# luuvish/arrow-h264

Measured on AMD Instinct MI355X. Metric: macroblocks/s (decode reconstruct, post-entropy) 1080p P-frame; % HBM roofline, higher is better.
Workload: dtype u8

## Files before the change

### arrow-h264_amd/csrc/k_deblock2.hip

```cpp
#include "kernels.h"
#include "mb_deblock.h"
#include "mb_deblock2.h"

using namespace h264r;

namespace {

constexpr int LPU = H264R_DB2_LPU;
static_assert(LPU == 4 || LPU == 8, "H264R_DB2_LPU");
constexpr int UNITS = DEBLOCK2_UNITS;
constexpr int NH = LPU / 4;
constexpr int BAND = H264R_DB2_BAND;
#ifndef H264R_DB2_PL
#define H264R_DB2_PL 2
#endif
constexpr int PL = H264R_DB2_PL;
constexpr bool DOY = PL != 1, DOC = PL != 0;
static_assert(PL == 2 || LPU == 8, "the split walk is built at 8 lanes per unit");
constexpr int PICS = UNITS / BAND;
#ifndef H264R_DB2_SG
#define H264R_DB2_SG 4
#endif
constexpr int SG = H264R_DB2_SG;
static_assert(SG == 4 || SG == 2, "H264R_DB2_SG");
static_assert(UNITS % BAND == 0, "a band divides the wave's units");
constexpr int RECG = 24;
static_assert(HANDOFF2_BYTES == 2 * RECG * sizeof(uint64_t), "the host sizes hb by HANDOFF2_BYTES per MB column");
constexpr int AUX_SC1 = 16;
constexpr int RSRC_W3 = 0x00020000;
constexpr uint32_t OOB = 0x80000000u;

constexpr int YR = DOY ? 16 : 0, CR = DOC ? 8 : 0;
struct alignas(16) UnitLds {
    uint32_t y[YR][8];
    uint32_t c[2][CR][4];
    uint32_t info[20];
};
static_assert(sizeof(UnitLds) == (PL == 2 ? 848 : PL == 0 ? 592 : 336), "UnitLds layout");

struct alignas(16) StageLds {
    uint32_t y[YR][SG][4];
    uint32_t c[2][CR][SG][2];
    uint32_t pad[SG == 4 ? 20 : 4];
};
static_assert(SG != 4 || sizeof(StageLds) == (PL == 2 ? 1616 : PL == 0 ? 1104 : 592), "StageLds layout");
struct alignas(16) UpLds {
    uint32_t yu[DOY ? 3 : 0][SG][4];
    uint32_t cu[2][DOC ? SG : 0][2];
};

typedef uint32_t v4u __attribute__((ext_vector_type(4)));
typedef uint32_t v2u __attribute__((ext_vector_type(2)));

DEV s2 unpack_cols(uint32_t w, int j) { return as_s2(__builtin_amdgcn_perm(w, w, 0x0C000C00u | ((uint32_t)(j + 2) << 16) | (uint32_t)j)); }
DEV uint32_t pack_cols(s2 c0, s2 c1) { return __builtin_amdgcn_perm(as_w(c1), as_w(c0), 0x06020400u); }
DEV s2 bs_pair(uint32_t w, int slo, int shi) { return (s2){(short)((w >> (8 * slo)) & 255), (short)((w >> (8 * shi)) & 255)}; }

template <int AUX = 0>
DEV void st16(__amdgpu_buffer_rsrc_t r, uint32_t off, v4u v)
{
    __builtin_amdgcn_raw_buffer_store_b128(__builtin_bit_cast(__attribute__((ext_vector_type(4))) unsigned int, v), r, off, 0, AUX);
}
template <int AUX = 0>
DEV void st8(__amdgpu_buffer_rsrc_t r, uint32_t off, v2u v)
{
    __builtin_amdgcn_raw_buffer_store_b64(__builtin_bit_cast(__attribute__((ext_vector_type(2))) unsigned int, v), r, off, 0, AUX);
}
template <int AUX = 0>
DEV void st4(__amdgpu_buffer_rsrc_t r, uint32_t off, uint32_t v) { __builtin_amdgcn_raw_buffer_store_b32(v, r, off, 0, AUX); }
#ifndef H264R_DB2_OUT_AUX
#define H264R_DB2_OUT_AUX 0
#endif
constexpr int OUT_AUX = H264R_DB2_OUT_AUX;

}

#ifndef H264R_DB2_KERNEL
#define H264R_DB2_KERNEL k_deblock2
#endif
#ifdef H264R_TRACE
#if H264R_DB2_PL == 0
#define h264r_db2_trace h264r_db2y_trace
#define h264r_db2_trace_copy h264r_db2y_trace_copy
#elif H264R_DB2_PL == 1
#define h264r_db2_trace h264r_db2c_trace
#define h264r_db2_trace_copy h264r_db2c_trace_copy
#endif
__device__ unsigned long long h264r_db2_trace[1 << 16][8];
#define TRACE(...) __VA_ARGS__
extern "C" void h264r_db2_trace_copy(void* dst) { (void)hipMemcpyFromSymbol(dst, HIP_SYMBOL(h264r_db2_trace), sizeof(h264r_db2_trace)); }
#else
#define TRACE(...)
#endif

#ifndef H264R_DB2_XCD
#define H264R_DB2_XCD 1
#endif
#ifndef H264R_DB2_DIAG
#define H264R_DB2_DIAG 0
#endif
#define H264R_DB2_WAVES_PER_EU (H264R_DB2_PL == 1 ? 4 : H264R_DB2_PL == 0 ? 3 : H264R_DB2_LPU == 8 ? (H264R_DB2_SG == 2 ? 3 : 2) : 1)
extern "C" __global__ __launch_bounds__(64) __attribute__((amdgpu_waves_per_eu(H264R_DB2_WAVES_PER_EU, H264R_DB2_WAVES_PER_EU))) void H264R_DB2_KERNEL(
    h264r_batch b, const DbInfo* __restrict__ dbinfo, uint64_t* hb, int* sync, int* err, uint32_t epoch, int2 rows, int nx,
    const uint8_t* __restrict__ recon)
{
    __shared__ UnitLds S[UNITS];
    __shared__ StageLds G[UNITS];
    __shared__ UpLds UP[PICS];
#ifdef H264R_DB2_LDS_PAD
    __shared__ uint32_t lds_pad[H264R_DB2_LDS_PAD / 4];
    if (threadIdx.x == 0 && epoch == 0xFFFFFFFFu) { lds_pad[0] = 1; __syncthreads(); err[0] = lds_pad[0]; }
#endif
    const Geom g = make_geom(b.width_mbs, b.height_mbs);
    const int W = g.wmb, R0 = rows.x, R1 = rows.y;
    const int ngroups = (b.num_pics + PICS - 1) / PICS;
    const int nbands = (R1 - R0 + BAND - 1) / BAND;
#if !H264R_DB2_XCD
    nx = 1;
#endif
    unsigned xcc_reg = 0;
    if (nx > 1) asm volatile("s_getreg_b32 %0, hwreg(HW_REG_XCC_ID)" : "=s"(xcc_reg));
    const int xcc = (int)(xcc_reg & 15u) % nx;
    const int ngx = (ngroups - xcc + nx - 1) / nx;
    int* counter = &sync[xcc];
    const bool local = nx > 1;
    const int items = ngx * nbands;
    for (;;) {
    __syncthreads();
    int tk = 0;
    if (threadIdx.x == 0) tk = atomicAdd(counter, 1);
    const int ticket = __builtin_amdgcn_readfirstlane(tk);
    if (ticket >= items) {
        xcd_drain_check(sync, sync + TICKET_DRAIN, nx, [&](int k) { return (ngroups - k + nx - 1) / nx * nbands; }, err);
        return;
    }
    const int band = ticket / ngx, grp = (ticket - band * ngx) * nx + xcc;
    int lane = threadIdx.x;
    asm volatile("" : "+v"(lane));
    const int u = lane / LPU, q8 = lane % LPU, q = q8 / NH, h = q8 % NH;
    const int rb = u / PICS, pu = u - rb * PICS;
    const int y = R0 + band * BAND + rb;
    const int pic0 = grp * PICS, npg = min(PICS, b.num_pics - pic0);
    const bool active = pu < npg && y < R1;
    const int pic = pic0 + min(pu, npg - 1), yc = min(y, R1 - 1);
    const bool above = y > R0, last_row = y == R1 - 1;
    const uint32_t tag32 = (epoch << 12) | ((uint32_t)band & 0xFFFu);
    const uint64_t tag_in = (uint64_t)((epoch << 12) | ((uint32_t)(band - 1) & 0xFFFu)) << 32;
    const bool polls = active && rb == 0 && above;
    const bool publishes = active && rb == BAND - 1 && !last_row;

    UnitLds& U = S[u];
    const UnitLds& A = S[rb ? u - PICS : u];
    StageLds& T = G[u];
    StageLds& TA = G[rb ? u - PICS : u];
    UpLds& TU = UP[pu];
    const uint32_t Wl = (uint32_t)g.W, Wc = (uint32_t)g.Wc;
    const uint32_t ysz = (uint32_t)g.ysz, csz = (uint32_t)g.csz;
    const __amdgpu_buffer_rsrc_t rY = __builtin_amdgcn_make_buffer_rsrc(b.out_y + (size_t)pic0 * g.ysz, 0, (int)(npg * ysz), RSRC_W3);
    const __amdgpu_buffer_rsrc_t rU = __builtin_amdgcn_make_buffer_rsrc(b.out_u + (size_t)pic0 * g.csz, 0, (int)(npg * csz), RSRC_W3);
    const __amdgpu_buffer_rsrc_t rV = __builtin_amdgcn_make_buffer_rsrc(b.out_v + (size_t)pic0 * g.csz, 0, (int)(npg * csz), RSRC_W3);
    const uint32_t yrow = active ? (uint32_t)(pic - pic0) * ysz + (uint32_t)y * 16u * Wl : OOB;
    const uint32_t crow = active ? (uint32_t)(pic - pic0) * csz + (uint32_t)y * 8u * Wc : OOB;
    const int p = q >> 1, d = q & 1;
    const v4u* info_row = reinterpret_cast<const v4u*>(dbinfo + (size_t)pic * g.nmb + (size_t)yc * W);
    const uint32_t hb_bytes = (uint32_t)b.num_pics * 2u * (uint32_t)W * RECG * 8u;
    const __amdgpu_buffer_rsrc_t hrs = __builtin_amdgcn_make_buffer_rsrc(hb, 0, (int)hb_bytes, RSRC_W3);
    const uint32_t rec_out = publishes ? (uint32_t)(((size_t)pic * 2 + (band & 1)) * W * RECG * 8) : OOB;
    const uint32_t rec_in = polls ? (uint32_t)(((size_t)pic * 2 + ((band + 1) & 1)) * W * RECG * 8) : OOB;
    constexpr uint64_t PAIR_POS = 0xba9654873210ull;
    auto pair_off = [&](uint32_t base, int m, int c, int k) -> uint32_t {
        const uint32_t bs = (uint32_t)(PAIR_POS >> (4 * (c * 3 + k))) & 15u;
        return base + (uint32_t)(m * RECG) * 8u + bs * 16u;
    };

    const uint8_t* rrow = recon + ((size_t)pic * g.nmb + (size_t)yc * W) * RECON_MB;
    constexpr int NLR = 16 / LPU, NCK = 8 / LPU;
    v4u wl[NLR], wc[NCK];
    auto fetch = [&](int m) {
#if H264R_DB2_DIAG & 2
        m = 0;
#endif
        const uint8_t* ma = rrow + (size_t)min(max(m, 0), W - 1) * RECON_MB;
        if constexpr (DOY) {
#pragma unroll
            for (int i = 0; i < NLR; ++i) wl[i] = load_global<v4u>(ma + (LPU * i + q8) * 16);
        }
        if constexpr (DOC) {
#pragma unroll
            for (int j = 0; j < NCK; ++j) wc[j] = load_global<v4u>(ma + RECON_CB + (LPU * j + q8) * 16);
        }
    };
    auto fill = [&](int s) {
        if constexpr (DOY) {
#pragma unroll
            for (int i = 0; i < NLR; ++i) *reinterpret_cast<v4u*>(&U.y[LPU * i + q8][4 * s]) = wl[i];
        }
#pragma unroll
        for (int j = 0; j < NCK; ++j) {
            const int k = LPU * j + q8, pl = k >> 2, r = 2 * (k & 3);
            if (DOC) {
                *reinterpret_cast<v2u*>(&U.c[pl][r][2 * s]) = wc[j].xy;
                *reinterpret_cast<v2u*>(&U.c[pl][r + 1][2 * s]) = wc[j].zw;
            }
        }
    };
    const int ylast = last_row || rb < BAND - 1 ? 15 : 12, clast = last_row || rb < BAND - 1 ? 7 : 6;
    auto stage_own = [&](int m, int s) {
        const int mc = max(m, 0);
        if constexpr (DOY) {
#pragma unroll
            for (int i = 0; i < NLR; ++i) {
                const int r = LPU * i + q8;
                *reinterpret_cast<v4u*>(&T.y[r][mc % SG][0]) = *reinterpret_cast<const v4u*>(&U.y[r][4 * s]);
            }
        }
        if constexpr (DOC) {
#pragma unroll
            for (int i = 0; i < NLR; ++i) {
                const int k = LPU * i + q8, pl = k >> 3, r = k & 7;
                *reinterpret_cast<v2u*>(&T.c[pl][r][mc % SG][0]) = *reinterpret_cast<const v2u*>(&U.c[pl][r][2 * s]);
            }
        }
    };
    auto store_groups = [&](int xs) {
        const int mo = xs - 1;
        const bool own = active && mo >= 0 && mo < W;
        const int r = lane / SG, pp = lane % SG, rr = min(r, 15), cp = rr >> 3, cr = rr & 7;
        for (uint64_t bm = __ballot(own && q8 == 0 && (mo % SG == SG - 1 || mo == W - 1)); bm; bm &= bm - 1) {
            const int l0 = __builtin_ctzll(bm), u2 = l0 / LPU;
            const int m2 = __builtin_amdgcn_readlane(mo, l0), yl2 = __builtin_amdgcn_readlane(ylast, l0);
            const int cl2 = __builtin_amdgcn_readlane(clast, l0);
            const uint32_t yr2 = (uint32_t)__builtin_amdgcn_readlane((int)yrow, l0);
            const uint32_t cr2 = (uint32_t)__builtin_amdgcn_readlane((int)crow, l0);
            const int g0 = m2 & ~(SG - 1);
            const bool inrow = g0 + pp <= m2 && r < 16;
            if constexpr (DOY)
                st16<OUT_AUX>(rY, r <= yl2 && inrow ? yr2 + (uint32_t)r * Wl + (uint32_t)(g0 + pp) * 16u : OOB,
                              *reinterpret_cast<const v4u*>(&G[u2].y[rr][pp][0]));
            if constexpr (DOC) {
                const uint32_t off = cr <= cl2 && inrow ? cr2 + (uint32_t)cr * Wc + (uint32_t)(g0 + pp) * 8u : OOB;
                const v2u cv = *reinterpret_cast<const v2u*>(&G[u2].c[cp][cr][pp][0]);
                st8<OUT_AUX>(rU, cp == 0 ? off : OOB, cv);
                st8<OUT_AUX>(rV, cp == 1 ? off : OOB, cv);
            }
        }
        const bool up = active && rb == 0 && above && xs >= 0 && xs < W;
        for (uint64_t bm = __ballot(up && q8 == 0 && (xs % SG == SG - 1 || xs == W - 1)); bm; bm &= bm - 1) {
            const int l0 = __builtin_ctzll(bm), pu2 = l0 / LPU;
            const int x2 = __builtin_amdgcn_readlane(xs, l0);
            const uint32_t yr2 = (uint32_t)__builtin_amdgcn_readlane((int)yrow, l0);
            const uint32_t cr2 = (uint32_t)__builtin_amdgcn_readlane((int)crow, l0);
            const int g0 = x2 & ~(SG - 1);
            const bool inrow = g0 + pp <= x2 && r < 16;
            if constexpr (DOY)
                st16<OUT_AUX>(rY, r < 3 && inrow ? yr2 - (uint32_t)(3 - r) * Wl + (uint32_t)(g0 + pp) * 16u : OOB,
                              *reinterpret_cast<const v4u*>(&UP[pu2].yu[min(r, 2)][pp][0]));
            if constexpr (DOC) {
                const uint32_t off = r < 2 && inrow ? cr2 - Wc + (uint32_t)(g0 + pp) * 8u : OOB;
                const v2u cv = *reinterpret_cast<const v2u*>(&UP[pu2].cu[r & 1][pp][0]);
                st8<OUT_AUX>(rU, r == 0 ? off : OOB, cv);
                st8<OUT_AUX>(rV, r == 1 ? off : OOB, cv);
            }
        }
    };
    auto granule = [&](int s, int c, int i) -> uint32_t {
        return i < 4 ? U.y[12 + i][4 * s + c] : U.c[c >> 1][2 + i][2 * s + (c & 1)];
    };
    auto publish_pair = [&](uint32_t base, int m, int s, int c, int k) {
        const v4u v = {granule(s, c, 2 * k), tag32, granule(s, c, 2 * k + 1), tag32};
        if (local) st16(hrs, pair_off(base, m, c, k), v);
        else st16<AUX_SC1>(hrs, pair_off(base, m, c, k), v);
    };
    auto early_c = [&](int lq, int j) { return lq < 3 ? (j ? 2 : 0) : 1; };
    auto early_k = [&](int lq, int j) { return lq < 3 ? lq : j; };
    auto late_c = [&](int lq) { return lq == 0 ? 1 : 3; };
    auto late_k = [&](int lq) { return lq == 0 ? 2 : lq - 1; };
    constexpr int NINF = LPU == 4 ? 2 : 1;
    v4u ninf[NINF];
    auto load_info = [&](int m) {
        const v4u* src = info_row + (size_t)min(max(m, 0), W - 1) * 5;
        ninf[0] = src[min(q8, 4)];
        if (NINF == 2) ninf[NINF - 1] = src[4];
    };
    auto put_info = [&](bool ok) {
        const v4u z = {0u, 0u, 0u, 0u};
        *reinterpret_cast<v4u*>(&U.info[4 * min(q8, 4)]) = ok ? ninf[0] : z;
        if (NINF == 2) *reinterpret_cast<v4u*>(&U.info[16]) = ok ? ninf[NINF - 1] : z;
    };
    auto partner = [&](uint32_t v) -> uint32_t {
        return (uint32_t)__builtin_amdgcn_update_dpp(0, (int)v, 0xB1, 0xF, 0xF, false);
    };

    TRACE(const unsigned long long tr_start = __builtin_amdgcn_s_memrealtime(); unsigned long long tph[4] = {0, 0, 0, 0};
          unsigned long long tm = __builtin_amdgcn_s_memtime();)
    bool ok = true;
    const int s0 = -2, s1 = W + BAND - 1;
    int x = s0 - rb;
    uint64_t rin[6];
    auto load_record = [&](int m) {
        const uint32_t base = active && m >= 0 && m < W ? rec_in : OOB;
#pragma unroll
        for (int k = PL == 1 ? 2 : 0; k < (PL == 0 ? 2 : 3); ++k) {
            const v4u v = __builtin_bit_cast(v4u, __builtin_amdgcn_raw_buffer_load_b128(hrs, pair_off(base, max(m, 0), q, k), 0, AUX_SC1));
            rin[2 * k] = v.x | (uint64_t)v.y << 32; rin[2 * k + 1] = v.z | (uint64_t)v.w << 32;
        }
    };
    put_info(false);
    wave_sync();
    fetch(x + 1);
    load_info(x + 1);
    for (int s = s0; s <= s1; ++s, ++x) {
        const bool xok = active && x >= 0 && x < W;
        const int sl = (x + 1) & 1, sc = x & 1;
        uint32_t inf[20];
#pragma unroll
        for (int k = 0; k < 5; ++k) {
            const v4u v = *reinterpret_cast<const v4u*>(&U.info[4 * k]);
            inf[4 * k] = v.x; inf[4 * k + 1] = v.y; inf[4 * k + 2] = v.z; inf[4 * k + 3] = v.w;
        }
        const uint32_t cpar[3] = {p ? inf[14] : inf[11], p ? inf[15] : inf[12], p ? inf[16] : inf[13]};

        {
          if constexpr (DOY) {
            EdgeP ev[4];
#pragma unroll
            for (int e = 0; e < 4; ++e) ev[e] = edge_params(inf[8 + (e == 0 ? 0 : 2)], bs_pair(inf[e], q, q));
#pragma unroll
            for (int ii = 0; ii < 2 / NH; ++ii) {
                const int i = NH == 2 ? h : ii;
                const int ra = 4 * q + i, rb2 = ra + 2;
                uint32_t la = U.y[ra][4 * sl + 3], lb = U.y[rb2][4 * sl + 3];
                const v4u Av = *reinterpret_cast<const v4u*>(&U.y[ra][4 * sc]);
                const v4u Bv = *reinterpret_cast<const v4u*>(&U.y[rb2][4 * sc]);
                uint32_t a[4] = {Av.x, Av.y, Av.z, Av.w}, bb[4] = {Bv.x, Bv.y, Bv.z, Bv.w};
                s2 c[20];
#pragma unroll
                for (int k = 0; k < 4; ++k) c[k] = unpack2(la, lb, k);
#pragma unroll
                for (int k = 4; k < 20; ++k) c[k] = unpack2(a[(k >> 2) - 1], bb[(k >> 2) - 1], k & 3);
                filter2<true, false>(c[0], c[1], c[2], c[3], c[4], c[5], c[6], c[7], ev[0]);
#pragma unroll
                for (int e = 1; e < 4; ++e)
                    filter2<false, false>(c[4 * e], c[4 * e + 1], c[4 * e + 2], c[4 * e + 3], c[4 * e + 4], c[4 * e + 5],
                                          c[4 * e + 6], c[4 * e + 7], ev[e]);
                pack4(c[0], c[1], c[2], c[3], la, lb);
#pragma unroll
                for (int k = 0; k < 4; ++k) pack4(c[4 + 4 * k], c[5 + 4 * k], c[6 + 4 * k], c[7 + 4 * k], a[k], bb[k]);
                U.y[ra][4 * sl + 3] = la;
                U.y[rb2][4 * sl + 3] = lb;
                *reinterpret_cast<v4u*>(&U.y[ra][4 * sc]) = (v4u){a[0], a[1], a[2], a[3]};
                *reinterpret_cast<v4u*>(&U.y[rb2][4 * sc]) = (v4u){bb[0], bb[1], bb[2], bb[3]};
            }
          }
            load_record(x);
          if constexpr (DOC) {
#pragma unroll
            for (int ii = 0; ii < 2 / NH; ++ii) {
                const int i = NH == 2 ? h : ii;
                const int ra = 4 * d + i, rb2 = ra + 2;
                EdgeP ec[2];
#pragma unroll
                for (int e = 0; e < 2; ++e)
                    ec[e] = edge_params(cpar[e == 0 ? 0 : 2], bs_pair(inf[2 * e], ra >> 1, rb2 >> 1));
                uint32_t la = U.c[p][ra][2 * sl + 1], lb = U.c[p][rb2][2 * sl + 1];
                const v2u Av = *reinterpret_cast<const v2u*>(&U.c[p][ra][2 * sc]);
                const v2u Bv = *reinterpret_cast<const v2u*>(&U.c[p][rb2][2 * sc]);
                uint32_t a[2] = {Av.x, Av.y}, bb[2] = {Bv.x, Bv.y};
                s2 c[12];
#pragma unroll
                for (int k = 0; k < 4; ++k) c[k] = unpack2(la, lb, k);
#pragma unroll
                for (int k = 4; k < 12; ++k) c[k] = unpack2(a[(k >> 2) - 1], bb[(k >> 2) - 1], k & 3);
                filter2<true, true>(c[0], c[1], c[2], c[3], c[4], c[5], c[6], c[7], ec[0]);
                filter2<false, true>(c[4], c[5], c[6], c[7], c[8], c[9], c[10], c[11], ec[1]);
                pack4(c[0], c[1], c[2], c[3], la, lb);
                pack4(c[4], c[5], c[6], c[7], a[0], bb[0]);
                pack4(c[8], c[9], c[10], c[11], a[1], bb[1]);
                U.c[p][ra][2 * sl + 1] = la;
                U.c[p][rb2][2 * sl + 1] = lb;
                *reinterpret_cast<v2u*>(&U.c[p][ra][2 * sc]) = (v2u){a[0], a[1]};
                *reinterpret_cast<v2u*>(&U.c[p][rb2][2 * sc]) = (v2u){bb[0], bb[1]};
            }
          }
        }
        TRACE({ const unsigned long long t2 = __builtin_amdgcn_s_memtime(); tph[0] += t2 - tm; tm = t2; })

        auto ready = [&]() {
            bool r = true;
#pragma unroll
            for (int i = PL == 1 ? 4 : 0; i < (PL == 0 ? 4 : 6); ++i) r &= (rin[i] & 0xFFFFFFFF00000000ull) == tag_in;
            return __builtin_amdgcn_readfirstlane(__all(r || !(polls && xok))) != 0;
        };
        if (!ready()) {
            WaitClock wclk;
            bool give_up = false;
            for (;;) {
                __builtin_amdgcn_s_sleep(1);
                load_record(x);
                if (ready()) break;
                if (wait_give_up(err, wclk)) { give_up = true; break; }
            }
            if (give_up) { ok = false; break; }
        }
        if (R0 > 0 && band == 0 && __builtin_amdgcn_readfirstlane(__any(rb == 0 && xok && inf[4] != 0)))
            __hip_atomic_store(err, DEV_ERR_BAND_EDGE, __ATOMIC_RELAXED, __HIP_MEMORY_SCOPE_AGENT);
        wave_sync();
        TRACE({ const unsigned long long t2 = __builtin_amdgcn_s_memtime(); tph[1] += t2 - tm; tm = t2; })
        if constexpr (PL == 2)
            publish_pair(active && x >= 1 && x <= W && h == 0 ? rec_out : OOB, max(x - 1, 0), sl, late_c(q), late_k(q));
        else if constexpr (PL == 0)
            publish_pair(active && x >= 1 && x <= W && q == 3 ? rec_out : OOB, max(x - 1, 0), sl, 3, h);
        else
            publish_pair(active && x >= 1 && x <= W && h == 0 && (q & 1) ? rec_out : OOB, max(x - 1, 0), sl, q, 2);
        if (rb) {
            if constexpr (DOY) {
#pragma unroll
                for (int r = 0; r < 4; ++r) rin[r] = A.y[12 + r][4 * sc + q];
            }
            if constexpr (DOC) {
#pragma unroll
                for (int r = 0; r < 2; ++r) rin[4 + r] = A.c[p][6 + r][2 * sc + d];
            }
        }
#if !(H264R_DB2_DIAG & 1)
        store_groups(x - 1);
        __builtin_amdgcn_fence(__ATOMIC_RELEASE, "wavefront");
#endif
        stage_own(x - 1, sl);
        wave_sync();
        fill(sl);
        put_info(active && x + 1 >= 0 && x + 1 < W);
        TRACE({ const unsigned long long t2 = __builtin_amdgcn_s_memtime(); tph[2] += t2 - tm; tm = t2; })

        uint32_t wy[20], wcv[10];
        {
        if constexpr (DOY) {
#pragma unroll
            for (int r = 0; r < 4; ++r) wy[r] = (uint32_t)rin[r];
#pragma unroll
            for (int r = 0; r < 16; ++r) wy[4 + r] = U.y[r][4 * sc + q];
            EdgeP eh[4];
#pragma unroll
            for (int e = 0; e < 4; ++e) eh[e] = edge_params(inf[8 + (e == 0 ? 1 : 2)], bs_pair(inf[4 + e], q, q));
            s2 c[2 / NH][20];
#pragma unroll
            for (int jj = 0; jj < 2 / NH; ++jj) {
                const int j = NH == 2 ? h : jj;
#pragma unroll
                for (int r = 0; r < 20; ++r) c[jj][r] = unpack_cols(wy[r], j);
                filter2<true, false>(c[jj][0], c[jj][1], c[jj][2], c[jj][3], c[jj][4], c[jj][5], c[jj][6], c[jj][7], eh[0]);
#pragma unroll
                for (int e = 1; e < 4; ++e)
                    filter2<false, false>(c[jj][4 * e], c[jj][4 * e + 1], c[jj][4 * e + 2], c[jj][4 * e + 3], c[jj][4 * e + 4],
                                          c[jj][4 * e + 5], c[jj][4 * e + 6], c[jj][4 * e + 7], eh[e]);
            }
#pragma unroll
            for (int r = 1; r < 20; ++r) {
                if constexpr (NH == 1) {
                    wy[r] = pack_cols(c[0][r], c[2 / NH - 1][r]);
                } else {
                    const s2 o = as_s2(partner(as_w(c[0][r])));
                    wy[r] = h ? pack_cols(o, c[0][r]) : pack_cols(c[0][r], o);
                }
            }
#pragma unroll
            for (int r = 0; r < 16; ++r) U.y[r][4 * sc + q] = wy[4 + r];
        }
        if constexpr (DOC) {
#pragma unroll
            for (int r = 0; r < 2; ++r) wcv[r] = (uint32_t)rin[4 + r];
#pragma unroll
            for (int r = 0; r < 8; ++r) wcv[2 + r] = U.c[p][r][2 * sc + d];
            EdgeP eh[2];
#pragma unroll
            for (int e = 0; e < 2; ++e) eh[e] = edge_params(cpar[e == 0 ? 1 : 2], bs_pair(inf[4 + 2 * e], 2 * d, 2 * d + 1));
            s2 c[2 / NH][10];
#pragma unroll
            for (int jj = 0; jj < 2 / NH; ++jj) {
                const int j = NH == 2 ? h : jj;
#pragma unroll
                for (int r = 0; r < 10; ++r) c[jj][r] = unpack_cols(wcv[r], j);
                s2 d0 = c[jj][0], d1 = c[jj][9];
                filter2<true, true>(d0, d0, c[jj][0], c[jj][1], c[jj][2], c[jj][3], d1, d1, eh[0]);
                filter2<false, true>(d0, d0, c[jj][4], c[jj][5], c[jj][6], c[jj][7], d1, d1, eh[1]);
            }
#pragma unroll
            for (int r = 1; r < 10; ++r) {
                if constexpr (NH == 1) {
                    wcv[r] = pack_cols(c[0][r], c[2 / NH - 1][r]);
                } else {
                    const s2 o = as_s2(partner(as_w(c[0][r])));
                    wcv[r] = h ? pack_cols(o, c[0][r]) : pack_cols(c[0][r], o);
                }
            }
#pragma unroll
            for (int r = 0; r < 8; ++r) U.c[p][r][2 * sc + d] = wcv[2 + r];
        }
        }

#pragma unroll
        for (int jj = 0; jj < 2 / NH; ++jj) {
            const int j = NH == 2 ? h : jj;
            if constexpr (PL == 2)
                publish_pair(xok ? rec_out : OOB, max(x, 0), sc, early_c(q, j), early_k(q, j));
            else if constexpr (PL == 0)
                publish_pair(xok && q < 3 ? rec_out : OOB, max(x, 0), sc, q, h);
            else
                publish_pair(xok && h == 0 && !(q & 1) ? rec_out : OOB, max(x, 0), sc, q, 2);
        }
        if (xok && above) {
            if constexpr (DOY) {
                uint32_t* yd = rb ? &TA.y[13][x % SG][q] : &TU.yu[0][x % SG][q];
#pragma unroll
                for (int r = 1; r < 4; ++r) yd[(r - 1) * 4 * SG] = wy[r];
            }
            if constexpr (DOC) *(rb ? &TA.c[p][7][x % SG][d] : &TU.cu[p][x % SG][d]) = wcv[1];
        }
        fetch(x + 2);
        load_info(x + 2);
        wave_sync();
        TRACE({ const unsigned long long t2 = __builtin_amdgcn_s_memtime(); tph[3] += t2 - tm; tm = t2; })
    }
#if !(H264R_DB2_DIAG & 1)
    if (ok) {
        wave_sync();
        store_groups(x - 1);
    }
#endif
    if (!ok) {
        for (int m = 0; m < W; ++m)
            for (int k = 0; k < 3; ++k) {
                const v4u v = {0u, tag32, 0u, tag32};
                if (local) st16(hrs, pair_off(rec_out, m, q, k), v);
                else st16<AUX_SC1>(hrs, pair_off(rec_out, m, q, k), v);
            }
    }
    TRACE(const int tix = band * ngroups + grp;
          if (lane == 0 && tix < (1 << 16)) {
        h264r_db2_trace[tix][0] = tr_start; h264r_db2_trace[tix][1] = __builtin_amdgcn_s_memrealtime();
        for (int i = 0; i < 4; ++i) h264r_db2_trace[tix][2 + i] = tph[i];
        h264r_db2_trace[tix][6] = (unsigned long long)W; })
    }
}
```

### arrow-h264_amd/csrc/mb_deblock2.h

```cpp
#pragma once
#include "device_common.h"

namespace h264r {

typedef short s2 __attribute__((ext_vector_type(2)));
typedef unsigned short u2 __attribute__((ext_vector_type(2)));

DEV s2 sp2(short v) { return (s2){v, v}; }
DEV s2 as_s2(uint32_t v) { return __builtin_bit_cast(s2, v); }
DEV uint32_t as_w(s2 v) { return __builtin_bit_cast(uint32_t, v); }
DEV s2 smin(s2 a, s2 b) { return __builtin_elementwise_min(a, b); }
DEV s2 smax(s2 a, s2 b) { return __builtin_elementwise_max(a, b); }
DEV s2 absd(s2 a, s2 b)
{
    const u2 ua = __builtin_bit_cast(u2, a), ub = __builtin_bit_cast(u2, b);
    return __builtin_bit_cast(s2, (u2)(__builtin_elementwise_max(ua, ub) - __builtin_elementwise_min(ua, ub)));
}
DEV s2 neg_mask(s2 v) { return v >> sp2(15); }
DEV s2 sel(s2 m, s2 a, s2 b)
{
    return as_s2((as_w(m) & as_w(a)) | (~as_w(m) & as_w(b)));
}
DEV s2 clamp255(s2 v) { return smin(smax(v, sp2(0)), sp2(255)); }
DEV s2 opaque_mask(s2 m)
{
    uint32_t w = as_w(m);
    asm volatile("" : "+v"(w));
    return as_s2(w);
}

DEV s2 unpack2(uint32_t A, uint32_t B, int b)
{
    return as_s2(__builtin_amdgcn_perm(B, A, 0x0C000C00u | ((uint32_t)(4 + b) << 16) | (uint32_t)b));
}
DEV void pack4(s2 c0, s2 c1, s2 c2, s2 c3, uint32_t& lo, uint32_t& hi)
{
    const uint32_t u = __builtin_amdgcn_perm(as_w(c1), as_w(c0), 0x06020400u);
    const uint32_t v = __builtin_amdgcn_perm(as_w(c3), as_w(c2), 0x06020400u);
    lo = __builtin_amdgcn_perm(v, u, 0x05040100u);
    hi = __builtin_amdgcn_perm(v, u, 0x07060302u);
}

DEV void merge2(s2 c0, s2 c1, int half, uint32_t& lo, uint32_t& hi)
{
    const uint32_t u = __builtin_amdgcn_perm(as_w(c1), as_w(c0), 0x06020400u);
    lo = __builtin_amdgcn_perm(lo, u, half ? 0x01000504u : 0x07060100u);
    hi = __builtin_amdgcn_perm(hi, u, half ? 0x03020504u : 0x07060302u);
}

struct EdgeP {
    s2 am1, bm1;
    s2 bs;
    s2 tc0;
    s2 alpha;
};

DEV EdgeP edge_params(uint32_t par, s2 bs2)
{
    EdgeP e;
    const short alpha = (short)(par & 255), beta = (short)((par >> 8) & 255);
    e.alpha = sp2(alpha);
    e.am1 = sp2((short)(alpha - 1));
    e.bm1 = sp2((short)(beta - 1));
    e.bs = bs2;
    const uint32_t T = (((par >> 16) & 31) << 8) | (((par >> 21) & 31) << 16) | (((par >> 26) & 31) << 24);
    e.tc0 = as_s2(__builtin_amdgcn_perm(0u, T, as_w(bs2) | 0x0c000c00u));
    return e;
}

template <bool STRONG, bool CHROMA>
DEV void filter2(s2& p3, s2& p2, s2& p1, s2& p0, s2& q0, s2& q1, s2& q2, s2& q3, const EdgeP& e)
{
    const s2 dpq = absd(p0, q0);
    const s2 nf = neg_mask(smin(smin(e.am1 - dpq, e.bm1 - absd(p1, p0)), smin(e.bm1 - absd(q1, q0), e.bs - sp2(1))));
    if (CHROMA) {
        const s2 tc = e.tc0 + sp2(1);
        s2 d = ((q0 - p0) * sp2(4) + (p1 - q1) + sp2(4)) >> sp2(3);
        d = smin(smax(d, -tc), tc);
        s2 np0 = clamp255(p0 + d), nq0 = clamp255(q0 - d);
        if (STRONG) {
            const s2 is4 = opaque_mask(neg_mask(e.bs - sp2(4)) ^ sp2(-1));
            np0 = sel(is4, (p1 * sp2(2) + p0 + q1 + sp2(2)) >> sp2(2), np0);
            nq0 = sel(is4, (q1 * sp2(2) + q0 + p1 + sp2(2)) >> sp2(2), nq0);
        }
        p0 = sel(nf, p0, np0);
        q0 = sel(nf, q0, nq0);
        return;
    }
    const s2 nap = neg_mask(e.bm1 - absd(p2, p0));
    const s2 naq = neg_mask(e.bm1 - absd(q2, q0));
    const s2 tc = e.tc0 + sp2(2) + nap + naq;
    s2 d = ((q0 - p0) * sp2(4) + (p1 - q1) + sp2(4)) >> sp2(3);
    d = smin(smax(d, -tc), tc);
    s2 np0 = clamp255(p0 + d), nq0 = clamp255(q0 - d);
    const s2 avg = (p0 + q0 + sp2(1)) >> sp2(1);
    s2 np1 = sel(nap, p1, p1 + smin(smax((p2 + avg - p1 * sp2(2)) >> sp2(1), -e.tc0), e.tc0));
    s2 nq1 = sel(naq, q1, q1 + smin(smax((q2 + avg - q1 * sp2(2)) >> sp2(1), -e.tc0), e.tc0));
    s2 np2 = p2, nq2 = q2;
    if (STRONG) {
        const s2 is4 = opaque_mask(neg_mask(e.bs - sp2(4)) ^ sp2(-1));
        const s2 nstrong = neg_mask(((e.alpha >> sp2(2)) + sp2(1)) - dpq);
        const s2 nsp = nap | nstrong, nsq = naq | nstrong;
        const s2 s_p0 = sel(nsp, (p1 * sp2(2) + p0 + q1 + sp2(2)) >> sp2(2),
                            (p2 + p1 * sp2(2) + p0 * sp2(2) + q0 * sp2(2) + q1 + sp2(4)) >> sp2(3));
        const s2 s_p1 = sel(nsp, p1, (p2 + p1 + p0 + q0 + sp2(2)) >> sp2(2));
        const s2 s_p2 = sel(nsp, p2, (p3 * sp2(2) + p2 * sp2(3) + p1 + p0 + q0 + sp2(4)) >> sp2(3));
        const s2 s_q0 = sel(nsq, (q1 * sp2(2) + q0 + p1 + sp2(2)) >> sp2(2),
                            (p1 + p0 * sp2(2) + q0 * sp2(2) + q1 * sp2(2) + q2 + sp2(4)) >> sp2(3));
        const s2 s_q1 = sel(nsq, q1, (p0 + q0 + q1 + q2 + sp2(2)) >> sp2(2));
        const s2 s_q2 = sel(nsq, q2, (q3 * sp2(2) + q2 * sp2(3) + q1 + q0 + p0 + sp2(4)) >> sp2(3));
        np0 = sel(is4, s_p0, np0); nq0 = sel(is4, s_q0, nq0);
        np1 = sel(is4, s_p1, np1); nq1 = sel(is4, s_q1, nq1);
        np2 = sel(is4, s_p2, p2);  nq2 = sel(is4, s_q2, q2);
        p2 = sel(nf, p2, np2);
        q2 = sel(nf, q2, nq2);
    }
    p1 = sel(nf, p1, np1);
    p0 = sel(nf, p0, np0);
    q0 = sel(nf, q0, nq0);
    q1 = sel(nf, q1, nq1);
}

}
```

Measured before the change: 766.6 million.

## Split horizontal-edge writeback into per-lane halves and tag bS with perm selectors

Adds a HALVES mode, on by default via STEP=9. In the 8-lanes-per-unit walk, each lane unpacks and writes back only its own 16-bit half of each column word with sub-dword LDS stores, where before both lanes exchanged and merged full words. It also builds boundary-strength pairs with a single v_perm using a tag byte set up once per lane, which replaces shift/mask extraction. Both are meant to cut VALU permute/merge work and LDS traffic in the per-macroblock loop. Other gated options (hoisting alpha/beta/tc0 parameters, precomputed edge constants) are plumbed but off by default, and the 16-bit LDS stores risk extra LDS store instructions and bank effects.

```diff
diff --git a/arrow-h264_amd/csrc/k_deblock2.hip b/arrow-h264_amd/csrc/k_deblock2.hip
--- a/arrow-h264_amd/csrc/k_deblock2.hip
+++ b/arrow-h264_amd/csrc/k_deblock2.hip
@@ -52,9 +52,23 @@
 typedef uint32_t v4u __attribute__((ext_vector_type(4)));
 typedef uint32_t v2u __attribute__((ext_vector_type(2)));
 
-DEV s2 unpack_cols(uint32_t w, int j) { return as_s2(__builtin_amdgcn_perm(w, w, 0x0C000C00u | ((uint32_t)(j + 2) << 16) | (uint32_t)j)); }
+constexpr bool HALVES = NH == 2 && (H264R_DB2_STEP & 1) != 0;
+DEV s2 unpack_cols(uint32_t w, int j)
+{
+    if constexpr (HALVES) return as_s2(__builtin_amdgcn_perm(w, w, 0x0C000C00u | ((uint32_t)(2 * j + 1) << 16) | (uint32_t)(2 * j)));
+    return as_s2(__builtin_amdgcn_perm(w, w, 0x0C000C00u | ((uint32_t)(j + 2) << 16) | (uint32_t)j));
+}
+typedef uint16_t __attribute__((may_alias)) u16_alias;
+DEV void store_half(uint32_t* dw, int h, s2 c)
+{
+    reinterpret_cast<u16_alias*>(dw)[h] = (uint16_t)__builtin_amdgcn_perm(as_w(c), as_w(c), 0x0C0C0200u);
+}
 DEV uint32_t pack_cols(s2 c0, s2 c1) { return __builtin_amdgcn_perm(as_w(c1), as_w(c0), 0x06020400u); }
-DEV s2 bs_pair(uint32_t w, int slo, int shi) { return (s2){(short)((w >> (8 * slo)) & 255), (short)((w >> (8 * shi)) & 255)}; }
+DEV s2 bs_pair(uint32_t w, int slo, int shi, uint32_t sel)
+{
+    if constexpr (DB2_BS_PERM) return bs_tagged(w, sel);
+    return (s2){(short)((w >> (8 * slo)) & 255), (short)((w >> (8 * shi)) & 255)};
+}
 
 template <int AUX = 0>
 DEV void st16(__amdgpu_buffer_rsrc_t r, uint32_t off, v4u v)
@@ -162,6 +176,9 @@
     const uint32_t yrow = active ? (uint32_t)(pic - pic0) * ysz + (uint32_t)y * 16u * Wl : OOB;
     const uint32_t crow = active ? (uint32_t)(pic - pic0) * csz + (uint32_t)y * 8u * Wc : OOB;
     const int p = q >> 1, d = q & 1;
+    const int hs0 = HALVES ? 2 * d + h : 2 * d, hs1 = HALVES ? 2 * d + h : 2 * d + 1;
+    const uint32_t bsel_y = pinned(bs_selector(q, q)), bsel_c = pinned(bs_selector(2 * d, 2 * d + 1));
+    const uint32_t bsel_ch = pinned(bs_selector(hs0, hs1));
     const v4u* info_row = reinterpret_cast<const v4u*>(dbinfo + (size_t)pic * g.nmb + (size_t)yc * W);
     const uint32_t hb_bytes = (uint32_t)b.num_pics * 2u * (uint32_t)W * RECG * 8u;
     const __amdgpu_buffer_rsrc_t hrs = __builtin_amdgcn_make_buffer_rsrc(hb, 0, (int)hb_bytes, RSRC_W3);
@@ -319,12 +336,14 @@
             inf[4 * k] = v.x; inf[4 * k + 1] = v.y; inf[4 * k + 2] = v.z; inf[4 * k + 3] = v.w;
         }
         const uint32_t cpar[3] = {p ? inf[14] : inf[11], p ? inf[15] : inf[12], p ? inf[16] : inf[13]};
+        [[maybe_unused]] const ParP py[3] = {par_params(inf[8]), par_params(inf[9]), par_params(inf[10])};
+        [[maybe_unused]] const ParP pc[3] = {par_params(cpar[0]), par_params(cpar[1]), par_params(cpar[2])};
 
         {
           if constexpr (DOY) {
             EdgeP ev[4];
 #pragma unroll
-            for (int e = 0; e < 4; ++e) ev[e] = edge_params(inf[8 + (e == 0 ? 0 : 2)], bs_pair(inf[e], q, q));
+            for (int e = 0; e < 4; ++e) ev[e] = edge_params<false>(py[e == 0 ? 0 : 2], bs_pair(inf[e], q, q, bsel_y));
 #pragma unroll
             for (int ii = 0; ii < 2 / NH; ++ii) {
                 const int i = NH == 2 ? h : ii;
@@ -361,7 +380,7 @@
                 EdgeP ec[2];
 #pragma unroll
                 for (int e = 0; e < 2; ++e)
-                    ec[e] = edge_params(cpar[e == 0 ? 0 : 2], bs_pair(inf[2 * e], ra >> 1, rb2 >> 1));
+                    ec[e] = edge_params<true>(pc[e == 0 ? 0 : 2], bs_pair(inf[2 * e], ra >> 1, rb2 >> 1, bsel_c));
                 uint32_t la = U.c[p][ra][2 * sl + 1], lb = U.c[p][rb2][2 * sl + 1];
                 const v2u Av = *reinterpret_cast<const v2u*>(&U.c[p][ra][2 * sc]);
                 const v2u Bv = *reinterpret_cast<const v2u*>(&U.c[p][rb2][2 * sc]);
@@ -433,6 +452,7 @@
         TRACE({ const unsigned long long t2 = __builtin_amdgcn_s_memtime(); tph[2] += t2 - tm; tm = t2; })
 
         uint32_t wy[20], wcv[10];
+        [[maybe_unused]] s2 hy[3], hc;
         {
         if constexpr (DOY) {
 #pragma unroll
@@ -441,7 +461,7 @@
             for (int r = 0; r < 16; ++r) wy[4 + r] = U.y[r][4 * sc + q];
             EdgeP eh[4];
 #pragma unroll
-            for (int e = 0; e < 4; ++e) eh[e] = edge_params(inf[8 + (e == 0 ? 1 : 2)], bs_pair(inf[4 + e], q, q));
+            for (int e = 0; e < 4; ++e) eh[e] = edge_params<false>(py[e == 0 ? 1 : 2], bs_pair(inf[4 + e], q, q, bsel_y));
             s2 c[2 / NH][20];
 #pragma unroll
             for (int jj = 0; jj < 2 / NH; ++jj) {
@@ -454,6 +474,12 @@
                     filter2<false, false>(c[jj][4 * e], c[jj][4 * e + 1], c[jj][4 * e + 2], c[jj][4 * e + 3], c[jj][4 * e + 4],
                                           c[jj][4 * e + 5], c[jj][4 * e + 6], c[jj][4 * e + 7], eh[e]);
             }
+            if constexpr (HALVES) {
+#pragma unroll
+                for (int r = 1; r < 4; ++r) hy[r - 1] = c[0][r];
+#pragma unroll
+                for (int r = 0; r < 14; ++r) store_half(&U.y[r][4 * sc + q], h, c[0][4 + r]);
+            } else {
 #pragma unroll
             for (int r = 1; r < 20; ++r) {
                 if constexpr (NH == 1) {
@@ -465,6 +491,7 @@
             }
 #pragma unroll
             for (int r = 0; r < 16; ++r) U.y[r][4 * sc + q] = wy[4 + r];
+            }
         }
         if constexpr (DOC) {
 #pragma unroll
@@ -473,7 +500,7 @@
             for (int r = 0; r < 8; ++r) wcv[2 + r] = U.c[p][r][2 * sc + d];
             EdgeP eh[2];
 #pragma unroll
-            for (int e = 0; e < 2; ++e) eh[e] = edge_params(cpar[e == 0 ? 1 : 2], bs_pair(inf[4 + 2 * e], 2 * d, 2 * d + 1));
+            for (int e = 0; e < 2; ++e) eh[e] = edge_params<true>(pc[e == 0 ? 1 : 2], bs_pair(inf[4 + 2 * e], hs0, hs1, bsel_ch));
             s2 c[2 / NH][10];
 #pragma unroll
             for (int jj = 0; jj < 2 / NH; ++jj) {
@@ -484,6 +511,12 @@
                 filter2<true, true>(d0, d0, c[jj][0], c[jj][1], c[jj][2], c[jj][3], d1, d1, eh[0]);
                 filter2<false, true>(d0, d0, c[jj][4], c[jj][5], c[jj][6], c[jj][7], d1, d1, eh[1]);
             }
+            if constexpr (HALVES) {
+                hc = c[0][1];
+                store_half(&U.c[p][0][2 * sc + d], h, c[0][2]);
+                store_half(&U.c[p][3][2 * sc + d], h, c[0][5]);
+                store_half(&U.c[p][4][2 * sc + d], h, c[0][6]);
+            } else {
 #pragma unroll
             for (int r = 1; r < 10; ++r) {
                 if constexpr (NH == 1) {
@@ -495,6 +528,7 @@
             }
 #pragma unroll
             for (int r = 0; r < 8; ++r) U.c[p][r][2 * sc + d] = wcv[2 + r];
+            }
         }
         }
 
@@ -512,9 +546,16 @@
             if constexpr (DOY) {
                 uint32_t* yd = rb ? &TA.y[13][x % SG][q] : &TU.yu[0][x % SG][q];
 #pragma unroll
-                for (int r = 1; r < 4; ++r) yd[(r - 1) * 4 * SG] = wy[r];
-            }
-            if constexpr (DOC) *(rb ? &TA.c[p][7][x % SG][d] : &TU.cu[p][x % SG][d]) = wcv[1];
+                for (int r = 1; r < 4; ++r) {
+                    if constexpr (HALVES) store_half(&yd[(r - 1) * 4 * SG], h, hy[r - 1]);
+                    else yd[(r - 1) * 4 * SG] = wy[r];
+                }
+            }
+            if constexpr (DOC) {
+                uint32_t* cd = rb ? &TA.c[p][7][x % SG][d] : &TU.cu[p][x % SG][d];
+                if constexpr (HALVES) store_half(cd, h, hc);
+                else *cd = wcv[1];
+            }
         }
         fetch(x + 2);
         load_info(x + 2);
diff --git a/arrow-h264_amd/csrc/mb_deblock2.h b/arrow-h264_amd/csrc/mb_deblock2.h
--- a/arrow-h264_amd/csrc/mb_deblock2.h
+++ b/arrow-h264_amd/csrc/mb_deblock2.h
@@ -48,38 +48,106 @@
     hi = __builtin_amdgcn_perm(hi, u, half ? 0x03020504u : 0x07060302u);
 }
 
+#ifndef H264R_DB2_STEP
+#define H264R_DB2_STEP 9
+#endif
+constexpr bool DB2_PAR_ONCE = (H264R_DB2_STEP & 2) != 0, DB2_EDGE_CONST = (H264R_DB2_STEP & 4) != 0;
+constexpr bool DB2_BS_PERM = (H264R_DB2_STEP & 8) != 0;
+
+DEV uint32_t pinned(uint32_t w)
+{
+    asm("" : "+v"(w));
+    return w;
+}
+DEV s2 pinned(s2 v) { return as_s2(pinned(as_w(v))); }
+
 struct EdgeP {
     s2 am1, bm1;
     s2 bs;
     s2 tc0;
     s2 alpha;
+    s2 bsm1;
+    s2 tcb;
+    s2 ntc0;
+    s2 a4;
 };
 
-DEV EdgeP edge_params(uint32_t par, s2 bs2)
+DEV uint32_t tc0_table(uint32_t par) { return (((par >> 16) & 31) << 8) | (((par >> 21) & 31) << 16) | (((par >> 26) & 31) << 24); }
+
+struct ParP {
+    uint32_t par;
+    s2 alpha, am1, bm1, a4;
+    uint32_t T;
+};
+DEV ParP par_params(uint32_t par)
+{
+    ParP pp;
+    pp.par = par;
+    if constexpr (DB2_PAR_ONCE) {
+        const short alpha = (short)(par & 255), beta = (short)((par >> 8) & 255);
+        pp.alpha = pinned(sp2(alpha));
+        pp.am1 = pinned(sp2((short)(alpha - 1)));
+        pp.bm1 = pinned(sp2((short)(beta - 1)));
+        pp.a4 = pinned(sp2((short)((alpha >> 2) + 1)));
+        pp.T = pinned(tc0_table(par));
+    }
+    return pp;
+}
+
+constexpr short BS_TAG = 0x0c00;
+DEV uint32_t bs_selector(int slo, int shi) { return 0x04000400u | (uint32_t)shi << 16 | (uint32_t)slo; }
+DEV s2 bs_tagged(uint32_t w, uint32_t selector)
+{
+    return as_s2(__builtin_amdgcn_perm(0x0c0c0c0cu, w, selector));
+}
+
+template <bool CHROMA>
+DEV EdgeP edge_params(const ParP& pp, s2 bs2)
 {
     EdgeP e;
-    const short alpha = (short)(par & 255), beta = (short)((par >> 8) & 255);
-    e.alpha = sp2(alpha);
-    e.am1 = sp2((short)(alpha - 1));
-    e.bm1 = sp2((short)(beta - 1));
-    e.bs = bs2;
-    const uint32_t T = (((par >> 16) & 31) << 8) | (((par >> 21) & 31) << 16) | (((par >> 26) & 31) << 24);
-    e.tc0 = as_s2(__builtin_amdgcn_perm(0u, T, as_w(bs2) | 0x0c000c00u));
+    uint32_t T;
+    if constexpr (DB2_PAR_ONCE) {
+        e.alpha = pp.alpha; e.am1 = pp.am1; e.bm1 = pp.bm1; e.a4 = pp.a4;
+        T = pp.T;
+    } else {
+        const short alpha = (short)(pp.par & 255), beta = (short)((pp.par >> 8) & 255);
+        e.alpha = sp2(alpha);
+        e.am1 = sp2((short)(alpha - 1));
+        e.bm1 = sp2((short)(beta - 1));
+        e.a4 = (e.alpha >> sp2(2)) + sp2(1);
+        T = tc0_table(pp.par);
+    }
+    if constexpr (DB2_BS_PERM) {
+        e.bs = bs2 - sp2(BS_TAG);
+        e.tc0 = as_s2(__builtin_amdgcn_perm(0u, T, as_w(bs2)));
+    } else {
+        e.bs = bs2;
+        e.tc0 = as_s2(__builtin_amdgcn_perm(0u, T, as_w(bs2) | 0x0c000c00u));
+    }
+    e.bsm1 = e.bs - sp2(1);
+    e.tcb = e.tc0 + sp2(CHROMA ? 1 : 2);
+    e.ntc0 = -e.tc0;
     return e;
+}
+
+DEV s2 bs4_mask(s2 bs)
+{
+    if constexpr (DB2_BS_PERM) return opaque_mask(neg_mask(sp2(3) - bs));
+    return opaque_mask(neg_mask(bs - sp2(4)) ^ sp2(-1));
 }
 
 template <bool STRONG, bool CHROMA>
 DEV void filter2(s2& p3, s2& p2, s2& p1, s2& p0, s2& q0, s2& q1, s2& q2, s2& q3, const EdgeP& e)
 {
     const s2 dpq = absd(p0, q0);
-    const s2 nf = neg_mask(smin(smin(e.am1 - dpq, e.bm1 - absd(p1, p0)), smin(e.bm1 - absd(q1, q0), e.bs - sp2(1))));
+    const s2 nf = neg_mask(smin(smin(e.am1 - dpq, e.bm1 - absd(p1, p0)), smin(e.bm1 - absd(q1, q0), DB2_EDGE_CONST ? e.bsm1 : e.bs - sp2(1))));
     if (CHROMA) {
-        const s2 tc = e.tc0 + sp2(1);
+        const s2 tc = DB2_EDGE_CONST ? e.tcb : e.tc0 + sp2(1);
         s2 d = ((q0 - p0) * sp2(4) + (p1 - q1) + sp2(4)) >> sp2(3);
         d = smin(smax(d, -tc), tc);
         s2 np0 = clamp255(p0 + d), nq0 = clamp255(q0 - d);
         if (STRONG) {
-            const s2 is4 = opaque_mask(neg_mask(e.bs - sp2(4)) ^ sp2(-1));
+            const s2 is4 = bs4_mask(e.bs);
             np0 = sel(is4, (p1 * sp2(2) + p0 + q1 + sp2(2)) >> sp2(2), np0);
             nq0 = sel(is4, (q1 * sp2(2) + q0 + p1 + sp2(2)) >> sp2(2), nq0);
         }
@@ -89,17 +157,18 @@
     }
     const s2 nap = neg_mask(e.bm1 - absd(p2, p0));
     const s2 naq = neg_mask(e.bm1 - absd(q2, q0));
-    const s2 tc = e.tc0 + sp2(2) + nap + naq;
+    const s2 tc = (DB2_EDGE_CONST ? e.tcb : e.tc0 + sp2(2)) + nap + naq;
     s2 d = ((q0 - p0) * sp2(4) + (p1 - q1) + sp2(4)) >> sp2(3);
     d = smin(smax(d, -tc), tc);
     s2 np0 = clamp255(p0 + d), nq0 = clamp255(q0 - d);
     const s2 avg = (p0 + q0 + sp2(1)) >> sp2(1);
-    s2 np1 = sel(nap, p1, p1 + smin(smax((p2 + avg - p1 * sp2(2)) >> sp2(1), -e.tc0), e.tc0));
-    s2 nq1 = sel(naq, q1, q1 + smin(smax((q2 + avg - q1 * sp2(2)) >> sp2(1), -e.tc0), e.tc0));
+    const s2 ntc0 = DB2_EDGE_CONST ? e.ntc0 : -e.tc0;
+    s2 np1 = sel(nap, p1, p1 + smin(smax((p2 + avg - p1 * sp2(2)) >> sp2(1), ntc0), e.tc0));
+    s2 nq1 = sel(naq, q1, q1 + smin(smax((q2 + avg - q1 * sp2(2)) >> sp2(1), ntc0), e.tc0));
     s2 np2 = p2, nq2 = q2;
     if (STRONG) {
-        const s2 is4 = opaque_mask(neg_mask(e.bs - sp2(4)) ^ sp2(-1));
-        const s2 nstrong = neg_mask(((e.alpha >> sp2(2)) + sp2(1)) - dpq);
+        const s2 is4 = bs4_mask(e.bs);
+        const s2 nstrong = neg_mask((DB2_EDGE_CONST ? e.a4 : (e.alpha >> sp2(2)) + sp2(1)) - dpq);
         const s2 nsp = nap | nstrong, nsq = naq | nstrong;
         const s2 s_p0 = sel(nsp, (p1 * sp2(2) + p0 + q1 + sp2(2)) >> sp2(2),
                             (p2 + p1 * sp2(2) + p0 * sp2(2) + q0 * sp2(2) + q1 + sp2(4)) >> sp2(3));
```

New measurement: 786.7 million, median of 6. 1.03x the previous value.
